# smithzvk/gsl-scattered-interpolation

Hardware: AMD Instinct MI355X
Metric: M interpolated points/sec (whole hot path: fill + solve + eval sweep per step) (higher is better)
Workload: dtype f64; 1 GPU; C3: 3-D N=16384 Gaussian RBF (16k x 16k fp64 Cholesky), M=1M targets per GPU; config=C3, n_centres=16384, dim=3, targets_per_gpu=1000000, targets_total=1000000, parallelism=1 GPU

## Files before the change

gsl-scattered-interpolation_amd/csrc/hip/chol.hip:

```cpp
#include "common.h"
#include <math.h>
#include <stdlib.h>

#ifdef SINTERP_DIAG_PROF
__device__ unsigned long long g_diag_ts[80];
#define TSTAMP(i) do { if (threadIdx.x == 0) g_diag_ts[i] = __builtin_readcyclecounter(); } while (0)
extern "C" int gsl_sinterp_hip_debug_diag_ts(unsigned long long *out) { return (int)hipMemcpyFromSymbol(out, HIP_SYMBOL(g_diag_ts), sizeof(unsigned long long) * 80); }
#endif
#include "chol_potrf.h"
#include "trsm128.h"



__global__ void __launch_bounds__(256)
chol_base_kernel(double *__restrict__ A, size_t lda, size_t n, size_t j0, int nb, int *__restrict__ info,
                 double *__restrict__ diag_store)
{
  __shared__ double sL[CB][CB + 1];
  __shared__ double sInv[CB];
  const int tid = threadIdx.x;

  const size_t row = j0 + nb + (size_t)blockIdx.x * blockDim.x + tid;
  double *p = A + row * lda + j0;
  double x[CB];
// ... 57 lines not shown
    x[j] = v * sInv[j];
  }
  if (vecrow) {
#pragma unroll
    for (int k = 0; k < CB; k += 2) *reinterpret_cast<double2 *>(p + k) = make_double2(x[k], x[k + 1]);
  } else {
#pragma unroll
    for (int k = 0; k < CB; k++) if (k < nb) p[k] = x[k];
  }
}

__global__ void __launch_bounds__(256)
chol_diag_writeback_kernel(double *__restrict__ A, size_t lda, size_t n, const double *__restrict__ diag_store)
{
  const size_t j0 = (size_t)blockIdx.x * CB;
  for (int e = threadIdx.x; e < CB * CB; e += 256) {
    const int r = e / CB, k = e % CB;
    if (k <= r && j0 + r < n) A[(j0 + r) * lda + j0 + k] = diag_store[(size_t)blockIdx.x * (CB * CB) + e];
  }
}


__global__ void __launch_bounds__(256)
chol_diag128_kernel(double *__restrict__ A, size_t lda, size_t j0, int *__restrict__ info, double *__restrict__ diag_store,
                    double *__restrict__ Dinvg, double *__restrict__ fb, size_t ldf, int nrhs)
{
  extern __shared__ __attribute__((aligned(16))) double sm[];
  chol_diag128_block<4>(sm, A + j0 * lda + j0, lda, j0, info, diag_store, Dinvg, fb, ldf, nrhs, threadIdx.x);
}

#define TRX 130
#define TRY 34
template <int RF>
__global__ void __launch_bounds__(256)
chol_trsm16_kernel(double *__restrict__ A, size_t lda, size_t n, size_t j0, const double *__restrict__ Dinvg, size_t row_start,
                   double *__restrict__ fb, size_t ldf, int nrhs)
{
  constexpr bool KSPLIT = RF == 1;
  constexpr int NP = KSPLIT ? 2 : 1;
  constexpr int NRF = KSPLIT ? 1 : RF / 2;
  constexpr int ROWS = 16 * RF;
  constexpr int LCH = KSPLIT ? 4 : 8;
  extern __shared__ __attribute__((aligned(16))) double sm[];
  double *Xp = sm;
  double *Yp = Xp + NP * ROWS * TRX;
  double *ys = Yp + NP * ROWS * TRY;
  const int tid = threadIdx.x, lane = tid & 63, wave = tid >> 6;
  const int f = wave & 1, g = wave >> 1, fr = lane & 15, fq = lane >> 4;
  const int plane = KSPLIT ? g : 0;
  const size_t row0 = row_start + (size_t)blockIdx.x * ROWS;
  const int dch = KSPLIT ? (f ? 4 : 2) : (f ? 8 : 4);
  const int dk0 = KSPLIT ? dch * g : 0, lk0 = KSPLIT ? 4 * g : 0;

  double a0[NRF][8], dv[4][8], lb[6][LCH], yv[3];
  double4_t cinit[NRF][3];
#pragma unroll
  for (int c = 0; c < 4; c++)
#pragma unroll
    for (int i = 0; i < 8; i++) dv[c][i] = i < dch ? Dinvg[c * 1024 + (16 * f + fr) * 32 + 4 * (dk0 + i) + fq] : 0.0;
#pragma unroll
  for (int c = 1; c < 4; c++)
#pragma unroll
    for (int p = 0; p < c; p++)
#pragma unroll
      for (int i = 0; i < LCH; i++)
        lb[c * (c - 1) / 2 + p][i] = A[(j0 + 32 * c + 16 * f + fr) * lda + j0 + 32 * p + 4 * (lk0 + i) + fq];
#pragma unroll
  for (int t = 0; t < NRF; t++) {
    const int rf = KSPLIT ? 0 : g + 2 * t;
    const size_t arow = row0 + 16 * rf + fr < n ? row0 + 16 * rf + fr : n - 1;
    const double *Arow = A + arow * lda + j0;
#pragma unroll
    for (int i = 0; i < 8; i++) a0[t][i] = i < dch ? Arow[4 * (dk0 + i) + fq] : 0.0;
#pragma unroll
    for (int c = 1; c < 4; c++)
#pragma unroll
      for (int rg = 0; rg < 4; rg++) {
        const size_t r = row0 + 16 * rf + fq + 4 * rg < n ? row0 + 16 * rf + fq + 4 * rg : n - 1;
        cinit[t][c - 1][rg] = plane == 0 ? A[r * lda + j0 + 32 * c + 16 * f + fr] : 0.0;
      }
  }
#pragma unroll
  for (int t = 0; t < 3; t++) { const int e = t * 256 + tid; yv[t] = e < nrhs * PB ? fb[(size_t)(e >> 7) * ldf + j0 + (e & 127)] : 0.0; }
#pragma unroll
  for (int t = 0; t < 3; t++) { const int e = t * 256 + tid; if (e < nrhs * PB) ys[e] = yv[t]; }

  double facc[RF][TRSV_MAXR];
#pragma unroll
  for (int t = 0; t < RF; t++)
#pragma unroll
    for (int q = 0; q < TRSV_MAXR; q++) facc[t][q] = 0.0;
  const int sr = tid >> 4, sc = (tid & 15) * 2;

#pragma unroll
  for (int c = 0; c < 4; c++) {
    if (c > 0) {
#pragma unroll
      for (int t = 0; t < NRF; t++) {
        const int rf = KSPLIT ? 0 : g + 2 * t;
        double4_t acc = cinit[t][c - 1];
#pragma unroll
        for (int p = 0; p < c; p++)
#pragma unroll
          for (int i = 0; i < LCH; i++) {
            const int k = 32 * p + 4 * (lk0 + i) + fq;
            double a = Xp[(16 * rf + fr) * TRX + k];
            if constexpr (KSPLIT) a += Xp[ROWS * TRX + (16 * rf + fr) * TRX + k];
            acc = __builtin_amdgcn_mfma_f64_16x16x4f64(-a, lb[c * (c - 1) / 2 + p][i], acc, 0, 0, 0);
          }
#pragma unroll
        for (int rg = 0; rg < 4; rg++) Yp[plane * ROWS * TRY + (16 * rf + fq + 4 * rg) * TRY + 16 * f + fr] = acc[rg];
      }
      __syncthreads();
    }
#pragma unroll
    for (int t = 0; t < NRF; t++) {
      const int rf = KSPLIT ? 0 : g + 2 * t;
      double4_t x = (double4_t){0.0, 0.0, 0.0, 0.0};
#pragma unroll
      for (int i = 0; i < 8; i++) {
        if (i < dch) {
          const int k = 4 * (dk0 + i) + fq;
          double a = a0[t][i];
          if (c > 0) {
            a = Yp[(16 * rf + fr) * TRY + k];
            if constexpr (KSPLIT) a += Yp[ROWS * TRY + (16 * rf + fr) * TRY + k];
          }
          x = __builtin_amdgcn_mfma_f64_16x16x4f64(a, dv[c][i], x, 0, 0, 0);
        }
      }
#pragma unroll
      for (int rg = 0; rg < 4; rg++) Xp[plane * ROWS * TRX + (16 * rf + fq + 4 * rg) * TRX + 32 * c + 16 * f + fr] = x[rg];
    }
    __syncthreads();
#pragma unroll
    for (int t = 0; t < RF; t++) {
      const int r = sr + 16 * t;
      double2 xv = *reinterpret_cast<const double2 *>(&Xp[r * TRX + 32 * c + sc]);
      if constexpr (KSPLIT) {
        const double2 x1 = *reinterpret_cast<const double2 *>(&Xp[ROWS * TRX + r * TRX + 32 * c + sc]);
        xv.x += x1.x; xv.y += x1.y;
      }
      const size_t grow = row0 + r;
      if (grow < n) *reinterpret_cast<double2 *>(A + grow * lda + j0 + 32 * c + sc) = xv;
#pragma unroll
      for (int q = 0; q < TRSV_MAXR; q++)
        if (q < nrhs) facc[t][q] = fma(xv.y, ys[q * PB + 32 * c + sc + 1], fma(xv.x, ys[q * PB + 32 * c + sc], facc[t][q]));
    }
  }
  if (nrhs > 0) {
#pragma unroll
    for (int t = 0; t < RF; t++) {
      const size_t grow = row0 + sr + 16 * t;
#pragma unroll
      for (int q = 0; q < TRSV_MAXR; q++) {
        if (q < nrhs) {
          double v = facc[t][q];
          v += __shfl_xor(v, 1);
          v += __shfl_xor(v, 2);
          v += __shfl_xor(v, 4);
          v += __shfl_xor(v, 8);
          if ((tid & 15) == 0 && grow < n) fb[(size_t)q * ldf + grow] -= v;
        }
      }
    }
  }
}

template <int RF>
static int launch_trsm16(gsl_sinterp_hip_ctx *ctx, double *A, size_t lda, size_t n, size_t j0, const double *d_linv, size_t row_start,
                         double *fb, size_t ldf, int nrhs)
{
  constexpr int NP = RF == 1 ? 2 : 1;
  const size_t lds = (size_t)(NP * 16 * RF * (TRX + TRY) + TRSV_MAXR * PB) * sizeof(double);
  { int ast = sinterp_func_lds(ctx, (const void *)chol_trsm16_kernel<RF>, (int)lds); if (ast) return ast; }
  const size_t below = n - row_start;
  hipLaunchKernelGGL(chol_trsm16_kernel<RF>, dim3((unsigned)((below + 16 * RF - 1) / (16 * RF))), dim3(256), lds, ctx->stream, A, lda, n, j0,
                     d_linv, row_start, fb, ldf, nrhs);
  return ST_SUCCESS;
}

__global__ void __launch_bounds__(256)
chol_trsm128_kernel(double *__restrict__ A, size_t lda, size_t n, size_t j0, const double *__restrict__ Dinvg, size_t row_start,
                    double *__restrict__ fb, size_t ldf, int nrhs)
{
  extern __shared__ __attribute__((aligned(16))) double sm[];
  double *Bt = sm;
  double *ys = sm + TRSM128_LDS;
  const int tid = threadIdx.x, lane = tid & 63, wave = tid >> 6;
  const int fr = lane & 15, fq = lane >> 4;
  const size_t row0 = row_start + (size_t)blockIdx.x * 64;
  double yv[3];
  trsm128_stage(sm, tid,
                [=](int r) { return A + (row0 + r < n ? row0 + r : n - 1) * lda + j0; },
                [=](int bi, int bj, int r, int k) { return A[(j0 + bi * 32 + r) * lda + j0 + bj * 32 + k]; },
                [=](int b, int r, int k) { return Dinvg[b * 1024 + r * 32 + k]; },
                [=, &yv] {
#pragma unroll
                  for (int t = 0; t < 3; t++) { const int e = t * 256 + tid; yv[t] = e < nrhs * PB ? fb[(size_t)(e >> 7) * ldf + j0 + (e & 127)] : 0.0; }
                });
#pragma unroll
  for (int t = 0; t < 3; t++) { const int e = t * 256 + tid; if (e < nrhs * PB) ys[e] = yv[t]; }
  __syncthreads();
  trsm128_solve(sm, tid, [=](int c, int f, int rg, double v) {
    const size_t grow = row0 + wave * 16 + fq + 4 * rg;
    if (grow < n) A[grow * lda + j0 + c * 32 + f * 16 + fr] = v;
  });
  if (nrhs > 0) {
    __syncthreads();
    const int r = tid >> 2, qd = tid & 3;
    const size_t grow = row0 + r;
    for (int q = 0; q < nrhs; q++) {
      double v = 0.0;
#pragma unroll
      for (int k = 0; k < 32; k++) v = fma(Bt[r * TR_LD + qd * 32 + k], ys[q * PB + qd * 32 + k], v);
      v += __shfl_xor(v, 1);
      v += __shfl_xor(v, 2);
      if (qd == 0 && grow < n) fb[(size_t)q * ldf + grow] -= v;
    }
  }
}


__global__ void __launch_bounds__(256)
tricpy_lower_to_upper_kernel(double *__restrict__ A, size_t lda, size_t n)
{
  __shared__ double tile[32][33];
  const size_t bi = blockIdx.y, bj = blockIdx.x;
  if (bj > bi) return;
  const int tx = threadIdx.x & 31, ty = threadIdx.x >> 5;
  for (int r = ty; r < 32; r += 8) {
    const size_t i = bi * 32 + r, j = bj * 32 + tx;
    tile[r][tx] = (i < n && j < n) ? A[i * lda + j] : 0.0;
  }
  __syncthreads();
  for (int r = ty; r < 32; r += 8) {
    const size_t j = bj * 32 + r, i = bi * 32 + tx;
    if (i < n && j < n && j < i) A[j * lda + i] = tile[tx][r];
  }
}

static size_t chol_split(size_t w)
{
  const size_t unit = w > PB ? PB : CB;
  size_t w1 = ((w / 2 + unit - 1) / unit) * unit;
  if (w1 >= w) w1 = w - unit;
  return w1;
}

static int g_chol_riders_last = 0;
extern "C" int gsl_sinterp_hip_debug_chol_riders(void) { return __atomic_load_n(&g_chol_riders_last, __ATOMIC_RELAXED); }

static bool chol_panel128_on(void) { return !SINTERP_ENV_ONCE("GSL_SINTERP_NO_PANEL128"); }

static bool chol_all128(size_t n, const double *d_a, size_t lda)
{
  return chol_panel128_on() && n % PB == 0 && (lda & 1) == 0 && ((((uintptr_t)d_a) & 15) == 0);
}

static bool chol_rider_applicable(bool all128, size_t n)
{
  return all128 && !SINTERP_ENV_ONCE("GSL_SINTERP_NO_DIAG_RIDER") && n >= 2 * PB;
}

static int chol_panel(gsl_sinterp_hip_ctx *ctx, double *A, size_t lda, size_t n, size_t j0, size_t w, int *d_info,
                      double *d_diag, double *fb, size_t ldf, int nrhs, unsigned *d_cnt, bool diag_done)
{
  int st;
  double *d_linv = d_diag + ((n + CB - 1) / CB) * (CB * CB);
  if (w == PB && chol_panel128_on() && (lda & 1) == 0 && ((((uintptr_t)(A + j0 * lda + j0)) & 15) == 0)) {
    const size_t lds_diag = DIAG128_LDS_BYTES;
    { int ast = sinterp_func_lds(ctx, (const void *)chol_diag128_kernel, (int)lds_diag); if (ast) return ast; }
    if (!diag_done)
      hipLaunchKernelGGL(chol_diag128_kernel, dim3(1), dim3(256), lds_diag, ctx->stream, A, lda, j0, d_info,
                         n % PB == 0 ? (double *)NULL : d_diag, d_linv, fb, ldf, nrhs);
    const size_t below = n - j0 - w;
    if (below) {
      static const int force_rf = sinterp_env_int("GSL_SINTERP_TRSM_RF", 0);
      int ast = 0;
      if (force_rf == 1 || (!force_rf && below <= 4096)) ast = launch_trsm16<1>(ctx, A, lda, n, j0, d_linv, j0 + PB, fb, ldf, nrhs);
      else if (force_rf == 2) ast = launch_trsm16<2>(ctx, A, lda, n, j0, d_linv, j0 + PB, fb, ldf, nrhs);
      else if (force_rf == 4) ast = launch_trsm16<4>(ctx, A, lda, n, j0, d_linv, j0 + PB, fb, ldf, nrhs);
      else {
        const size_t lds_trsm = (size_t)(TRSM128_LDS + TRSV_MAXR * PB) * sizeof(double);
        ast = sinterp_func_lds(ctx, (const void *)chol_trsm128_kernel, (int)lds_trsm);
        if (!ast)
          hipLaunchKernelGGL(chol_trsm128_kernel, dim3((unsigned)((below + 63) / 64)), dim3(256), lds_trsm, ctx->stream, A, lda, n, j0,
                             (const double *)d_linv, j0 + PB, fb, ldf, nrhs);
      }
      if (ast) return ast;
    }
    LAUNCH_CHECK(ctx);
    return ST_SUCCESS;
  }
  if (w <= PB) {
    if (diag_done) return sinterp_fail(ctx, ST_EFAILED, "cholesky: rider on a panel that is not 128 wide", hipSuccess, __FILE__, __LINE__);
    if (fb) return sinterp_fail(ctx, ST_EFAILED, "cholesky: folded forward substitution on a panel that is not 128 wide", hipSuccess, __FILE__, __LINE__);
  }
  if (w <= CB) {
    const size_t below = n - j0 - w;
    const unsigned grid = (unsigned)((below + 255) / 256) + (below == 0 ? 1u : 0u);
// ... 317 lines not shown
  __shared__ double sx[TRSV_MAXR][TS];
  __shared__ double sb[TRSV_MAXR][TS];
  __shared__ double sW[TS][TS + 1];
  const int tid = threadIdx.x, lane = tid & 63, wave = tid >> 6;

  double t[16];
  size_t irow = 0;
  bool have = false;
  const int rsub = lane >> 3, c8 = (lane & 7) * 8;
  if (mode == 1) {
    irow = (size_t)blockIdx.x * 64 + lane;
    have = irow < j0;
#pragma unroll
    for (int jj = 0; jj < 16; jj++)
      t[jj] = (have && wave * 16 + jj < nb) ? T[(j0 + wave * 16 + jj) * ldt + irow] : 0.0;
  } else {
    const size_t base = (mode == 0) ? j0 + nb : 0;
    const size_t limit = (mode == 0) ? n : j0;
#pragma unroll
    for (int pass = 0; pass < 2; pass++) {
      const size_t i = base + ((size_t)blockIdx.x * 2 + pass) * 32 + wave * 8 + rsub;
      const double *row = T + i * ldt + j0 + c8;
#pragma unroll
      for (int k = 0; k < 8; k++) t[pass * 8 + k] = (i < limit && c8 + k < nb) ? row[k] : 0.0;
    }
  }
  const double *D = Dinv + (j0 / TS) * (size_t)(TS * TS);
  for (int e = tid; e < TS * TS; e += 256) {
    const int r = e / TS, c = e % TS;
    sW[r][c] = D[e];
  }
  for (int e = tid; e < nrhs * TS; e += 256) {
    const int r = e / TS, c = e % TS;
    sb[r][c] = c < nb ? b[r * ldb + j0 + c] : 0.0;
  }
  __syncthreads();
  for (int r = wave; r < nrhs; r += 4) {
    double acc = 0.0;
    if (mode == 0) { for (int c = 0; c < TS; c++) acc = fma(sW[lane][c], sb[r][c], acc); }
    else { for (int c = 0; c < TS; c++) acc = fma(sW[c][lane], sb[r][c], acc); }
    sx[r][lane] = acc;
    if (blockIdx.x == 0 && lane < nb) xout[r * ldb + j0 + lane] = acc;
  }
  __syncthreads();
  if (mode == 1) {
    __shared__ double s_part[TRSV_MAXR][4][64];
#pragma unroll
    for (int r = 0; r < TRSV_MAXR; r++) {
      if (r < nrhs) {
        double acc = 0.0;
#pragma unroll
        for (int jj = 0; jj < 16; jj++) acc = fma(t[jj], sx[r][wave * 16 + jj], acc);
        s_part[r][wave][lane] = acc;
      }
    }
    __syncthreads();
    if (wave == 0 && have) {
#pragma unroll
      for (int r = 0; r < TRSV_MAXR; r++)
        if (r < nrhs) b[r * ldb + irow] -= (s_part[r][0][lane] + s_part[r][1][lane]) + (s_part[r][2][lane] + s_part[r][3][lane]);
    }
  } else {
    const size_t base = (mode == 0) ? j0 + nb : 0;
    const size_t limit = (mode == 0) ? n : j0;
#pragma unroll
    for (int pass = 0; pass < 2; pass++) {
      const size_t i = base + ((size_t)blockIdx.x * 2 + pass) * 32 + wave * 8 + rsub;
#pragma unroll
      for (int r = 0; r < TRSV_MAXR; r++) {
        if (r < nrhs) {
          double a = 0.0;
#pragma unroll
          for (int k = 0; k < 8; k++) a = fma(t[pass * 8 + k], sx[r][c8 + k], a);
          a += __shfl_xor(a, 1);
          a += __shfl_xor(a, 2);
          a += __shfl_xor(a, 4);
          if (i < limit && (lane & 7) == 0) b[r * ldb + i] -= a;
        }
      }
    }
  }
}

__global__ void __launch_bounds__(256)
trsv_dataflow_kernel(const double *__restrict__ T, size_t ldt, size_t n, const double *__restrict__ b, double *xout, size_t ldb,
                     int nrhs, int mode, const double *__restrict__ Dinv, unsigned *tf, unsigned long long *xq, unsigned nblk)
{
  const unsigned want = __hip_atomic_load(tf, __ATOMIC_RELAXED, __HIP_MEMORY_SCOPE_AGENT) + 1u;
  const size_t npad = (size_t)nblk * TS;
  __shared__ double sx[2][TRSV_MAXR][TS];
  __shared__ double sW[TS][TS + 1];
  __shared__ double srhs[TRSV_MAXR][TS];
  __shared__ double s_part[TRSV_MAXR][4][TS];
  const int tid = threadIdx.x, lane = tid & 63, wave = tid >> 6;
  const int rsub = lane >> 3, c8 = (lane & 7) * 8;
  for (unsigned t = blockIdx.x; t < nblk; t += gridDim.x) {
    const unsigned I = (mode == 0) ? t : nblk - 1 - t;
    const size_t i0 = (size_t)I * TS;
    const int nbI = (int)((n - i0) < TS ? (n - i0) : TS);
    __syncthreads();
    for (int e = tid; e < TS * TS; e += 256) sW[e / TS][e % TS] = Dinv[(size_t)I * (TS * TS) + e];
    double bpre[(TRSV_MAXR * TS + 255) / 256];
#pragma unroll
    for (int q = 0; q < (TRSV_MAXR * TS + 255) / 256; q++) {
      const int e = q * 256 + tid, r = e / TS, c = e % TS;
      bpre[q] = (e < nrhs * TS && c < nbI) ? b[r * ldb + i0 + c] : 0.0;
    }
    double acc[TRSV_MAXR][2];
#pragma unroll
    for (int r = 0; r < TRSV_MAXR; r++) acc[r][0] = acc[r][1] = 0.0;
    for (unsigned sstep = 0; sstep < t; sstep++) {
      const unsigned J = (mode == 0) ? sstep : nblk - 1 - sstep;
      const size_t j0 = (size_t)J * TS;
      double tt[16];
      if (mode == 1) {
#pragma unroll
        for (int jj = 0; jj < 16; jj++) {
          const size_t jr = j0 + wave * 16 + jj;
          tt[jj] = (jr < n && lane < nbI) ? T[jr * ldt + i0 + lane] : 0.0;
        }
      } else {
#pragma unroll
        for (int pass = 0; pass < 2; pass++) {
          const size_t i = i0 + pass * 32 + wave * 8 + rsub;
          const double *row = T + i * ldt + j0 + c8;
          if (i < n && j0 + TS <= n && ((((uintptr_t)row) & 15) == 0)) {
#pragma unroll
            for (int k = 0; k < 8; k += 2) { const double2 v = *reinterpret_cast<const double2 *>(row + k); tt[pass * 8 + k] = v.x; tt[pass * 8 + k + 1] = v.y; }
          } else {
#pragma unroll
            for (int k = 0; k < 8; k++) tt[pass * 8 + k] = (i < n && j0 + c8 + k < n) ? row[k] : 0.0;
          }
        }
      }
      const int buf = sstep & 1;
      for (int e = tid; e < nrhs * TS; e += 256) {
        const int r = e / TS, c = e % TS;
        double v = 0.0;
        if (j0 + c < n) {
          const unsigned long long *q = xq + 2 * ((size_t)r * npad + j0 + c);
          unsigned long long w0, w1;
          for (;;) {
            w0 = __hip_atomic_load(q, __ATOMIC_RELAXED, __HIP_MEMORY_SCOPE_AGENT);
            w1 = __hip_atomic_load(q + 1, __ATOMIC_RELAXED, __HIP_MEMORY_SCOPE_AGENT);
            if ((unsigned)(w0 >> 32) == want && (unsigned)(w1 >> 32) == want) break;
            __builtin_amdgcn_s_sleep(1);
          }
          v = __hiloint2double((int)(unsigned)w1, (int)(unsigned)w0);
        }
        sx[buf][r][c] = v;
      }
      __syncthreads();
      if (mode == 1) {
#pragma unroll
        for (int r = 0; r < TRSV_MAXR; r++)
          if (r < nrhs) {
#pragma unroll
            for (int jj = 0; jj < 16; jj++) acc[r][0] = fma(tt[jj], sx[buf][r][wave * 16 + jj], acc[r][0]);
          }
      } else {
#pragma unroll
        for (int r = 0; r < TRSV_MAXR; r++)
          if (r < nrhs) {
#pragma unroll
            for (int pass = 0; pass < 2; pass++)
#pragma unroll
              for (int k = 0; k < 8; k++) acc[r][pass] = fma(tt[pass * 8 + k], sx[buf][r][c8 + k], acc[r][pass]);
          }
      }
    }
    if (mode == 1) {
#pragma unroll
      for (int r = 0; r < TRSV_MAXR; r++) if (r < nrhs) s_part[r][wave][lane] = acc[r][0];
      __syncthreads();
#pragma unroll
      for (int q = 0; q < (TRSV_MAXR * TS + 255) / 256; q++) {
        const int e = q * 256 + tid, r = e / TS, c = e % TS;
        if (e < nrhs * TS) {
          const double sum = (s_part[r][0][c] + s_part[r][1][c]) + (s_part[r][2][c] + s_part[r][3][c]);
          srhs[r][c] = (c < nbI) ? bpre[q] - sum : 0.0;
        }
      }
    } else {
#pragma unroll
      for (int r = 0; r < TRSV_MAXR; r++)
        if (r < nrhs) {
#pragma unroll
          for (int pass = 0; pass < 2; pass++) {
            double a = acc[r][pass];
            a += __shfl_xor(a, 1);
            a += __shfl_xor(a, 2);
            a += __shfl_xor(a, 4);
            const int row = pass * 32 + wave * 8 + rsub;
            if ((lane & 7) == 0) srhs[r][row] = -a;
          }
        }
      __syncthreads();
#pragma unroll
      for (int q = 0; q < (TRSV_MAXR * TS + 255) / 256; q++) {
        const int e = q * 256 + tid, r = e / TS, c = e % TS;
        if (e < nrhs * TS) srhs[r][c] = (c < nbI) ? bpre[q] + srhs[r][c] : 0.0;
      }
    }
    __syncthreads();
    for (int r = wave; r < nrhs; r += 4) {
      double p0 = 0.0, p1 = 0.0, p2 = 0.0, p3 = 0.0;
      if (mode == 0) {
#pragma unroll
        for (int c = 0; c < TS; c += 4) {
          p0 = fma(sW[lane][c], srhs[r][c], p0); p1 = fma(sW[lane][c + 1], srhs[r][c + 1], p1);
          p2 = fma(sW[lane][c + 2], srhs[r][c + 2], p2); p3 = fma(sW[lane][c + 3], srhs[r][c + 3], p3);
        }
      } else {
#pragma unroll
        for (int c = 0; c < TS; c += 4) {
          p0 = fma(sW[c][lane], srhs[r][c], p0); p1 = fma(sW[c + 1][lane], srhs[r][c + 1], p1);
          p2 = fma(sW[c + 2][lane], srhs[r][c + 2], p2); p3 = fma(sW[c + 3][lane], srhs[r][c + 3], p3);
        }
      }
      if (lane < nbI) {
        const double xv = (p0 + p1) + (p2 + p3);
        unsigned long long *q = xq + 2 * ((size_t)r * npad + i0 + lane);
        const unsigned long long tag = (unsigned long long)want << 32;
        __hip_atomic_store(q, tag | (unsigned)__double2loint(xv), __ATOMIC_RELAXED, __HIP_MEMORY_SCOPE_AGENT);
        __hip_atomic_store(q + 1, tag | (unsigned)__double2hiint(xv), __ATOMIC_RELAXED, __HIP_MEMORY_SCOPE_AGENT);
        xout[r * ldb + i0 + lane] = xv;
      }
    }
    if (t == nblk - 1) {
      __syncthreads();
      if (tid == 0) __hip_atomic_store(tf, want, __ATOMIC_RELAXED, __HIP_MEMORY_SCOPE_AGENT);
    }
  }
}

static int trsv_launches(gsl_sinterp_hip_ctx *ctx, size_t n, const double *T, size_t ldt, double *b, double *xout,
                         size_t ldb, int nrhs, int mode, int unit, double *d_inv, int inv_ready)
{
  const size_t nblk = (n + TS - 1) / TS;
  const bool use_inv = nblk > 1 && d_inv != NULL;
  if (use_inv && !inv_ready) {
    hipLaunchKernelGGL(tri_inv_kernel, dim3((unsigned)nblk), dim3(64), 0, ctx->stream, T, ldt, n, mode == 2 ? 1 : 0, unit, d_inv);
    LAUNCH_CHECK(ctx);
  }
  const bool no_df = SINTERP_ENV_ONCE("GSL_SINTERP_NO_DATAFLOW_TRSV");
  if (use_inv && !no_df && ctx->sk_wgs > 0 && ctx->d_tf && ctx->tf_count >= nblk + 1 && ctx->d_xq) {
    const unsigned G = (unsigned)(nblk < (size_t)ctx->sk_wgs ? nblk : (size_t)ctx->sk_wgs);
    hipLaunchKernelGGL(trsv_dataflow_kernel, dim3(G), dim3(256), 0, ctx->stream, T, ldt, n, (const double *)b, xout, ldb, nrhs, mode,
                       (const double *)d_inv, ctx->d_tf, ctx->d_xq, (unsigned)nblk);
    LAUNCH_CHECK(ctx);
    return ST_SUCCESS;
  }
  for (size_t t = 0; t < nblk; t++) {
    const size_t blk = (mode == 0) ? t : nblk - 1 - t;
    const size_t j0 = blk * TS;
    const int nb = (int)((n - j0) < TS ? (n - j0) : TS);
    const size_t rest = (mode == 0) ? n - j0 - nb : j0;
    const unsigned grid = (unsigned)((rest + 63) / 64);
    if (use_inv)
      hipLaunchKernelGGL(trsv_sweep_inv_kernel, dim3(grid ? grid : 1), dim3(256), 0, ctx->stream, T, ldt, n, b, xout, ldb, nrhs,
                         j0, nb, mode, (const double *)d_inv);
    else
      hipLaunchKernelGGL(trsv_sweep_kernel, dim3(grid ? grid : 1), dim3(256), 0, ctx->stream, T, ldt, n, b, xout, ldb, nrhs, j0,
                         nb, mode, unit);
    LAUNCH_CHECK(ctx);
  }
  return ST_SUCCESS;
}

__global__ void __launch_bounds__(256)
vec_copy_kernel(const double *__restrict__ src, double *__restrict__ dst, size_t count)
{
  const size_t i = (size_t)blockIdx.x * 256 + threadIdx.x;
  if (i < count) dst[i] = src[i];
}

static int trsv_multi_ex(gsl_sinterp_hip_ctx *ctx, size_t n, const double *T, size_t ldt, double *b, double *xout, size_t ldb,
                         int nrhs, int mode, int unit, int inv_ready)
{
  if (n == 0 || nrhs == 0) return ST_SUCCESS;
  if (nrhs > TRSV_MAXR) return sinterp_fail(ctx, ST_EINVAL, "trsv: too many right-hand sides", hipSuccess, __FILE__, __LINE__);
  const int slot = mode == 0 ? 2 : 3;
  const sinterp_graph_key gkey = {{n, ldt, (uintptr_t)T, (uintptr_t)b, (uintptr_t)xout, ldb, (uintptr_t)nrhs, (uintptr_t)mode,
                                    (uintptr_t)unit, (uintptr_t)inv_ready}};
  int replayed = 0;
  int st = sinterp_graph_try_launch(ctx, slot, gkey, &replayed);
  if (st || replayed) return st;
  void *d_inv = NULL;
  const size_t inv_bytes = ((n + TS - 1) / TS) * TS * TS * sizeof(double);
  const bool in_place = b == xout;
  if (in_place && inv_ready) return sinterp_fail(ctx, ST_EINVAL, "trsv: in-place sweep cannot reuse inverted blocks", hipSuccess, __FILE__, __LINE__);
  st = sinterp_invbuf(ctx, inv_bytes + (in_place ? (size_t)nrhs * ldb * sizeof(double) : 0), &d_inv);
  if (st) return st;
  {
    const size_t need = (n + TS - 1) / TS + 1;
    if (need > ctx->tf_count) {
      HIP_OK(ctx, hipStreamSynchronize(ctx->stream));
      if (ctx->d_tf) { HIP_OK(ctx, hipFree(ctx->d_tf)); ctx->d_tf = NULL; ctx->tf_count = 0; }
      const size_t cnt = need < 1024 ? 1024 : need * 2;
      HIP_OK(ctx, hipMalloc((void **)&ctx->d_tf, cnt * sizeof(unsigned)));
      HIP_OK(ctx, hipMemset(ctx->d_tf, 0, cnt * sizeof(unsigned)));
      if (ctx->d_xq) { HIP_OK(ctx, hipFree(ctx->d_xq)); ctx->d_xq = NULL; }
      const size_t xq_bytes = (size_t)TRSV_MAXR * cnt * TS * 2 * sizeof(unsigned long long);
      HIP_OK(ctx, hipMalloc((void **)&ctx->d_xq, xq_bytes));
      HIP_OK(ctx, hipMemset(ctx->d_xq, 0, xq_bytes));
      HIP_OK(ctx, hipDeviceSynchronize());
      ctx->tf_count = cnt;
      for (int i = 2; i < 4; i++)
        if (ctx->graph[i].exec) { (void)hipGraphExecDestroy(ctx->graph[i].exec); ctx->graph[i].exec = NULL; }
    }
  }
  st = sinterp_streamk_prepare(ctx);
  if (st) return st;
  double *b_src = in_place ? (double *)((char *)d_inv + inv_bytes) : b;
  hipStream_t saved;
  st = sinterp_capture_begin(ctx, &saved);
  if (st) return st;
  if (in_place) {
    const size_t cnt = (size_t)(nrhs - 1) * ldb + n;
    hipLaunchKernelGGL(vec_copy_kernel, dim3((unsigned)((cnt + 255) / 256)), dim3(256), 0, ctx->stream, (const double *)b, b_src, cnt);
  }
  st = trsv_launches(ctx, n, T, ldt, b_src, xout, ldb, nrhs, mode, unit, (double *)d_inv, inv_ready);
  int st2 = sinterp_capture_end(ctx, saved, slot, gkey);
  return st ? st : st2;
}

int sinterp_trsv_multi(gsl_sinterp_hip_ctx *ctx, size_t n, const double *T, size_t ldt, double *b, double *xout, size_t ldb,
                       int nrhs, int mode, int unit)
{
  return trsv_multi_ex(ctx, n, T, ldt, b, xout, ldb, nrhs, mode, unit, 0);
}

int sinterp_trsv(gsl_sinterp_hip_ctx *ctx, size_t n, const double *T, size_t ldt, double *b, double *xout, int mode,
                 int unit)
{
  return sinterp_trsv_multi(ctx, n, T, ldt, b, xout, n, 1, mode, unit);
}

int sinterp_cholesky_svx_multi(gsl_sinterp_hip_ctx *ctx, size_t n, const double *d_llt, size_t lda, double *d_x, size_t ldx,
                               int nrhs)
{
  EXCLUSIVE_SECTION(ctx);
  void *d_tmp = NULL;
  int st = sinterp_workspace(ctx, (size_t)nrhs * ldx * sizeof(double), &d_tmp);
  if (st) return st;
  st = sinterp_trsv_multi(ctx, n, d_llt, lda, d_x, (double *)d_tmp, ldx, nrhs, 0, 0);
  if (st) return st;
  return trsv_multi_ex(ctx, n, d_llt, lda, (double *)d_tmp, d_x, ldx, nrhs, 1, 0, 1);
}

extern "C" int gsl_sinterp_hip_cholesky_svx(gsl_sinterp_hip_ctx *ctx, size_t n, const double *d_llt, size_t lda, double *d_x)
{
  REQUIRE(ctx, ctx != NULL, ST_EFAULT);
  HIP_OK(ctx, hipSetDevice(ctx->device));
  EXCLUSIVE_SECTION(ctx);
  REQUIRE(ctx, lda >= n, ST_EINVAL);
  REQUIRE(ctx, n == 0 || (d_llt && d_x), ST_EFAULT);
  return sinterp_cholesky_svx_multi(ctx, n, d_llt, lda, d_x, n, 1);
}
```

gsl-scattered-interpolation_amd/csrc/hip/chol_potrf.h:

```cpp
#ifndef SINTERP_CHOL_POTRF_H
#define SINTERP_CHOL_POTRF_H

#define CB 32
#ifndef TSTAMP
#define TSTAMP(i) do { } while (0)
#endif
#if defined(SINTERP_DIAG_PROF_COLS)
#define TSTAMP_COL(i) TSTAMP(i)
#else
#define TSTAMP_COL(i) do { } while (0)
#endif

__device__ __forceinline__ double lane_bcast(double v, int src)
{
  int lo = __builtin_amdgcn_readlane(__double2loint(v), src);
  int hi = __builtin_amdgcn_readlane(__double2hiint(v), src);
  return __hiloint2double(hi, lo);
}

typedef double double4_t __attribute__((ext_vector_type(4)));
#define PB 128
#define PQ 34
#define PBLK (32 * PQ)
#define TR_LD 130
// ... 27 lines not shown
#define PIN_SSV(x, y, z)   asm volatile("" : "+s"(x), "+s"(y), "+v"(z) : : "memory")
#define PIN_SV(x, y)       asm volatile("" : "+s"(x), "+v"(y) : : "memory")

#define HB 16
template <int K0, int J>
__device__ __forceinline__ void potrf32_step(double (&a)[CB], double vprev, double cur, double inv_prev, double e, double e2, double q,
                                             const double *D, double *colp, const double (&rp)[CB])
{
  constexpr int END = K0 + HB;
  if constexpr (J < END) {
    TSTAMP_COL(32 + J);
    double v, d, uL2 = 0.0, acol = 0.0;
    if constexpr (J == K0) {
      v = cur;
      d = lane_bcast(v, J);
    } else {
      const double uL = e * inv_prev;
      d = fma(-uL, uL, q);
      acol = vprev * inv_prev;
      v = fma(-acol, uL, cur);
      uL2 = e2 * inv_prev;
    }
    double y0 = __builtin_amdgcn_rsq(d);
    PIN_V4(y0, v, uL2, acol);
    if constexpr (J > K0) { a[J - 1] = acol; colp[J - 1] = acol; }
    double rn[CB];
    if constexpr (J + 2 < END) {
#pragma unroll
      for (int k = K0; k < J; k += 2) {
        const double2 t2 = *reinterpret_cast<const double2 *>(D + (J + 2) * PQ + k);
        rn[k] = t2.x;
        if (k + 1 < CB) rn[k + 1] = t2.y;
      }
    }
    double en = 0.0, e2n = 0.0, qn = 0.0, curn = 0.0;
    if constexpr (J + 1 < END) en = lane_bcast(v, J + 1);
    if constexpr (J + 2 < END) e2n = lane_bcast(v, J + 2);
    if constexpr (J + 1 < END) {
      double p0 = a[J + 1], p1 = 0.0;
      if constexpr (J >= K0 + 1) p1 = -acol * uL2;
      PIN_SSV(en, e2n, p0);
#pragma unroll
      for (int k = K0; k + 1 < J; k++) {
        if (k & 1) p1 = fma(-a[k], rp[k], p1);
        else p0 = fma(-a[k], rp[k], p0);
      }
      curn = (J >= K0 + 1) ? p0 + p1 : p0;
      qn = lane_bcast(curn, J + 1);
      PIN_SV(qn, y0);
    }
    const double t = d * y0;
    const double rr = fma(-t, y0, 1.0);
    const double s1 = fma(0.375, rr, 0.5), u = y0 * rr;
    const double inv = fma(u, s1, y0);
    potrf32_step<K0, J + 1>(a, v, curn, inv, en, e2n, qn, D, colp, rn);
  } else {
    a[END - 1] = vprev * inv_prev;
    colp[END - 1] = a[END - 1];
  }
}

__device__ __forceinline__ void potrf32_split(double *D, double *Dt, int lane)
{
  const int fr = lane & 15, fq = lane >> 4;
  const double *ap = D + (HB + fr) * PQ + fq;
  const double *bp = Dt + fr * PQ + fq;
  double4_t cu, cw = (double4_t){0.0, 0.0, 0.0, 0.0};
#pragma unroll
  for (int rg = 0; rg < 4; rg++) cu[rg] = D[(HB + fq + 4 * rg) * PQ + HB + fr];
#pragma unroll
  for (int kk = 0; kk < 4; kk++) {
    const double av = ap[kk * 4], na = -av;
    cu = __builtin_amdgcn_mfma_f64_16x16x4f64(na, av, cu, 0, 0, 0);
    cw = __builtin_amdgcn_mfma_f64_16x16x4f64(na, bp[kk * 4], cw, 0, 0, 0);
  }
#pragma unroll
  for (int rg = 0; rg < 4; rg++) {
    D[(HB + fq + 4 * rg) * PQ + HB + fr] = cu[rg];
    Dt[fr * PQ + HB + fq + 4 * rg] = cw[rg];
  }
}


template <int NW>
__device__ __forceinline__ void potrf128_lds(double *S, double *Dv, int tid, int *__restrict__ info, size_t j0)
{
  const int lane = tid & 63, wave = tid >> 6;
  auto potrf_block = [&](int jb) {
    double *D = S + pblk(jb, jb);
    const bool is_row = lane < CB;
    double *Dt = Dv + jb * PBLK;
    double *colp = is_row ? D + lane * PQ : Dt + (lane - CB) * PQ;
    double a[CB];
#pragma unroll
    for (int k = 0; k < CB; k += 2) { const double2 t = *reinterpret_cast<const double2 *>(colp + k); a[k] = t.x; a[k + 1] = t.y; }
    double r0[CB];
    potrf32_step<0, 0>(a, 0.0, a[0], 0.0, 0.0, 0.0, 0.0, D, colp, r0);
    potrf32_split(D, Dt, lane);
#pragma unroll
    for (int k = HB; k < CB; k += 2) { const double2 t = *reinterpret_cast<const double2 *>(colp + k); a[k] = t.x; a[k + 1] = t.y; }
    potrf32_step<HB, HB>(a, 0.0, a[HB], 0.0, 0.0, 0.0, 0.0, D, colp, r0);
    const double dg = D[(lane & (CB - 1)) * PQ + (lane & (CB - 1))];
    const unsigned long long badm = __ballot(is_row && !(dg > 0.0));
    if (badm && lane == 0) atomicCAS(info, 0, (int)(j0 + jb * 32 + __ffsll((long long)badm)));
  };
  auto update_frag = [&](int jb, int bi, int bj, int f) {
    double *Cb = S + pblk(bi, bj);
    double4_t c = frag_load(Cb, f >> 1, f & 1, lane);
    c = frag_nt(S + pblk(bi, jb), S + pblk(bj, jb), f >> 1, f & 1, lane, c, -1.0);
    frag_store(Cb, f >> 1, f & 1, lane, c);
  };

  for (int jb = -1; jb < 3; jb++) {
    if (jb >= 0) {
    for (int u = wave; u < (3 - jb) * 2; u += NW) {
      double *Bb = S + pblk(jb + 1 + (u >> 1), jb);
      const int fi = u & 1;
      const double *ap = Bb + (fi * 16 + (lane & 15)) * PQ + (lane >> 4);
      const double *bp = Dv + jb * PBLK + (lane >> 4) * PQ + (lane & 15);
      double4_t x0 = (double4_t){0.0, 0.0, 0.0, 0.0}, x1 = x0;
#pragma unroll
      for (int kk = 0; kk < 8; kk++) {
        const double av = ap[kk * 4];
        if (kk < 4) x0 = __builtin_amdgcn_mfma_f64_16x16x4f64(av, bp[kk * 4 * PQ], x0, 0, 0, 0);
        x1 = __builtin_amdgcn_mfma_f64_16x16x4f64(av, bp[kk * 4 * PQ + 16], x1, 0, 0, 0);
      }
      frag_store(Bb, fi, 0, lane, x0);
      frag_store(Bb, fi, 1, lane, x1);
    }
    __syncthreads();
    TSTAMP(4 + jb * 4);
    if (wave < 3) update_frag(jb, jb + 1, jb + 1, wave == 0 ? 0 : wave + 1);
    __syncthreads();
    TSTAMP(5 + jb * 4);
    }
    if (wave == 0) {
      potrf_block(jb + 1);
    } else if (jb >= 0) {
      int unit = 0;
      for (int bi = jb + 2; bi < 4; bi++)
        for (int bj = jb + 1; bj <= bi; bj++)
          for (int f = 0; f < 4; f++) {
            if (bi == bj && f == 1) continue;
            if (unit++ % (NW - 1) == wave - 1) update_frag(jb, bi, bj, f);
          }
    }
    __syncthreads();
    TSTAMP(6 + jb * 4);
  }

}

#ifndef TRSV_MAXR
#define TRSV_MAXR 5
#endif

template <int NW>
__device__ __forceinline__ void diag128_forward(const double *S, const double *Dv, double *fs, double *tt, int tid, int nrhs)
{
  const int lane = tid & 63, wave = tid >> 6, r = lane & 31, half = lane >> 5;
  for (int q = wave; q < nrhs; q += NW) {
    double *y = fs + q * PB, *t = tt + q * CB;
#pragma unroll
    for (int i = 0; i < 4; i++) {
      double sum = 0.0;
#pragma unroll
      for (int kb = 0; kb < i; kb++) {
        const double *Lr = S + pblk(i, kb) + r * PQ + half * 16;
        const double *yk = y + kb * 32 + half * 16;
#pragma unroll
        for (int k = 0; k < 16; k += 2) {
          const double2 l2 = *reinterpret_cast<const double2 *>(Lr + k);
          sum = fma(l2.x, yk[k], sum);
          sum = fma(l2.y, yk[k + 1], sum);
        }
      }
      sum += __shfl_xor(sum, 32);
      if (half == 0) t[r] = y[i * 32 + r] - sum;
      __builtin_amdgcn_wave_barrier();
      const double *Wr = Dv + i * PBLK + (half * 16) * PQ + r;
      double acc = 0.0;
#pragma unroll
      for (int c = 0; c < 16; c++) acc = fma(Wr[c * PQ], t[half * 16 + c], acc);
      acc += __shfl_xor(acc, 32);
      if (half == 0) y[i * 32 + r] = acc;
      __builtin_amdgcn_wave_barrier();
    }
  }
}

#define DIAG128_LDS_BYTES ((size_t)(14 * PBLK + TRSV_MAXR * (PB + CB)) * sizeof(double))

template <int NW>
__device__ __forceinline__ void chol_diag128_block(double *sm, double *Ab, size_t lda, size_t j0, int *info, double *diag_store,
                                                   double *Dinvg, double *fb, size_t ldf, int nrhs, int tid)
{
  constexpr int NT = NW * 64;
  constexpr int RP = NT / 32;
  constexpr int PS = 32 / RP;
  constexpr int FT = (TRSV_MAXR * PB + NT - 1) / NT;
  static_assert(RP * PS == 32, "threads per workgroup");
  double *S = sm;
  double *Dv = S + 10 * PBLK;
  double *fs = Dv + 4 * PBLK;
  double *tt = fs + TRSV_MAXR * PB;
  TSTAMP(0);

  {
    double v[10 * PS], fv[FT];
    const int r8 = tid >> 5, k = tid & 31;
#pragma unroll
    for (int t = 0; t < 10 * PS; t++) {
      constexpr int BI[10] = {0, 1, 1, 2, 2, 2, 3, 3, 3, 3}, BJ[10] = {0, 0, 1, 0, 1, 2, 0, 1, 2, 3};
      const int b = t / PS, r = (t % PS) * RP + r8;
      v[t] = Ab[(size_t)(BI[b] * 32 + r) * lda + BJ[b] * 32 + k];
    }
#pragma unroll
    for (int t = 0; t < FT; t++) { const int e = t * NT + tid; fv[t] = e < nrhs * PB ? fb[(size_t)(e >> 7) * ldf + j0 + (e & 127)] : 0.0; }
#pragma unroll
    for (int t = 0; t < 10 * PS; t++) S[(t / PS) * PBLK + ((t % PS) * RP + r8) * PQ + k] = v[t];
#pragma unroll
    for (int t = 0; t < 4 * PS; t++) { const int r = (t % PS) * RP + r8; Dv[(t / PS) * PBLK + r * PQ + k] = r == k ? 1.0 : 0.0; }
#pragma unroll
    for (int t = 0; t < FT; t++) { const int e = t * NT + tid; if (e < nrhs * PB) fs[e] = fv[t]; }
  }
  __syncthreads();
  TSTAMP(1);

  potrf128_lds<NW>(S, Dv, tid, info, j0);

  TSTAMP(18);
  if (nrhs > 0) {
    diag128_forward<NW>(S, Dv, fs, tt, tid, nrhs);
    __syncthreads();
  }
  {
    const int r8 = tid >> 5, k = tid & 31;
#pragma unroll
    for (int t = 0; t < 10 * PS; t++) {
      constexpr int BI[10] = {0, 1, 1, 2, 2, 2, 3, 3, 3, 3}, BJ[10] = {0, 0, 1, 0, 1, 2, 0, 1, 2, 3};
      const int b = t / PS, r = (t % PS) * RP + r8, bi = BI[b], bj = BJ[b];
      const double v = S[b * PBLK + r * PQ + k];
      if (bi != bj || k <= r) Ab[(size_t)(bi * 32 + r) * lda + bj * 32 + k] = v;
      if (bi == bj && diag_store) diag_store[(j0 / CB + bi) * (CB * CB) + r * CB + k] = (k <= r) ? v : 0.0;
    }
#pragma unroll
    for (int t = 0; t < 4 * PS; t++) {
      const int b = t / PS, r = (t % PS) * RP + r8;
      Dinvg[b * 1024 + r * 32 + k] = Dv[b * PBLK + k * PQ + r];
    }
#pragma unroll
    for (int t = 0; t < FT; t++) { const int e = t * NT + tid; if (e < nrhs * PB) fb[(size_t)(e >> 7) * ldf + j0 + (e & 127)] = fs[e]; }
  }
  TSTAMP(19);
}

#endif
```

Measured before the change: 33.21 M points/s.

## Overlap diagonal forward solve with potrf and prefetch RHS in trsm kernels

Interleaves the per-block forward substitution for the right-hand sides into the potrf128 pipeline, so idle waves run it while wave 0 factors the next diagonal block. The trsm16 and trsm128 kernels now prefetch the RHS values early and write them back directly instead of doing a read-modify-write at the end. The in-place vector copy is skipped when the dataflow TRSV path applies. The dataflow kernel also gains a bounded spin with an abort flag that writes NaN if polling times out. This adds complexity and ties correctness to the abort_word scratch slot and the removed __restrict__ on b.

```diff
diff --git a/gsl-scattered-interpolation_amd/csrc/hip/chol.hip b/gsl-scattered-interpolation_amd/csrc/hip/chol.hip
--- a/gsl-scattered-interpolation_amd/csrc/hip/chol.hip
+++ b/gsl-scattered-interpolation_amd/csrc/hip/chol.hip
@@ -163,6 +163,12 @@
   }
 #pragma unroll
   for (int t = 0; t < 3; t++) { const int e = t * 256 + tid; yv[t] = e < nrhs * PB ? fb[(size_t)(e >> 7) * ldf + j0 + (e & 127)] : 0.0; }
+  double fv[RF][TRSV_MAXR];
+#pragma unroll
+  for (int t = 0; t < RF; t++)
+#pragma unroll
+    for (int q = 0; q < TRSV_MAXR; q++)
+      fv[t][q] = ((tid & 15) == 0 && q < nrhs && row0 + (tid >> 4) + 16 * t < n) ? fb[(size_t)q * ldf + row0 + (tid >> 4) + 16 * t] : 0.0;
 #pragma unroll
   for (int t = 0; t < 3; t++) { const int e = t * 256 + tid; if (e < nrhs * PB) ys[e] = yv[t]; }
 
@@ -241,7 +247,7 @@
           v += __shfl_xor(v, 2);
           v += __shfl_xor(v, 4);
           v += __shfl_xor(v, 8);
-          if ((tid & 15) == 0 && grow < n) fb[(size_t)q * ldf + grow] -= v;
+          if ((tid & 15) == 0 && grow < n) fb[(size_t)q * ldf + grow] = fv[t][q] - v;
         }
       }
     }
@@ -272,13 +278,17 @@
   const int fr = lane & 15, fq = lane >> 4;
   const size_t row0 = row_start + (size_t)blockIdx.x * 64;
   double yv[3];
+  double fv[TRSV_MAXR];
+  const bool fown = (tid & 3) == 0 && row0 + (tid >> 2) < n;
   trsm128_stage(sm, tid,
                 [=](int r) { return A + (row0 + r < n ? row0 + r : n - 1) * lda + j0; },
                 [=](int bi, int bj, int r, int k) { return A[(j0 + bi * 32 + r) * lda + j0 + bj * 32 + k]; },
                 [=](int b, int r, int k) { return Dinvg[b * 1024 + r * 32 + k]; },
-                [=, &yv] {
+                [=, &yv, &fv] {
 #pragma unroll
                   for (int t = 0; t < 3; t++) { const int e = t * 256 + tid; yv[t] = e < nrhs * PB ? fb[(size_t)(e >> 7) * ldf + j0 + (e & 127)] : 0.0; }
+#pragma unroll
+                  for (int q = 0; q < TRSV_MAXR; q++) fv[q] = (fown && q < nrhs) ? fb[(size_t)q * ldf + row0 + (tid >> 2)] : 0.0;
                 });
 #pragma unroll
   for (int t = 0; t < 3; t++) { const int e = t * 256 + tid; if (e < nrhs * PB) ys[e] = yv[t]; }
@@ -291,13 +301,16 @@
     __syncthreads();
     const int r = tid >> 2, qd = tid & 3;
     const size_t grow = row0 + r;
-    for (int q = 0; q < nrhs; q++) {
-      double v = 0.0;
-#pragma unroll
-      for (int k = 0; k < 32; k++) v = fma(Bt[r * TR_LD + qd * 32 + k], ys[q * PB + qd * 32 + k], v);
-      v += __shfl_xor(v, 1);
-      v += __shfl_xor(v, 2);
-      if (qd == 0 && grow < n) fb[(size_t)q * ldf + grow] -= v;
+#pragma unroll
+    for (int q = 0; q < TRSV_MAXR; q++) {
+      if (q < nrhs) {
+        double v = 0.0;
+#pragma unroll
+        for (int k = 0; k < 32; k++) v = fma(Bt[r * TR_LD + qd * 32 + k], ys[q * PB + qd * 32 + k], v);
+        v += __shfl_xor(v, 1);
+        v += __shfl_xor(v, 2);
+        if (fown) fb[(size_t)q * ldf + grow] = fv[q] - v;
+      }
     }
   }
 }
@@ -781,9 +794,11 @@
   }
 }
 
+#define TRSV_MAX_POLLS (1u << 22)
 __global__ void __launch_bounds__(256)
-trsv_dataflow_kernel(const double *__restrict__ T, size_t ldt, size_t n, const double *__restrict__ b, double *xout, size_t ldb,
-                     int nrhs, int mode, const double *__restrict__ Dinv, unsigned *tf, unsigned long long *xq, unsigned nblk)
+trsv_dataflow_kernel(const double *__restrict__ T, size_t ldt, size_t n, const double *b, double *xout, size_t ldb,
+                     int nrhs, int mode, const double *__restrict__ Dinv, unsigned *tf, unsigned long long *xq, unsigned nblk,
+                     unsigned *abort_word)
 {
   const unsigned want = __hip_atomic_load(tf, __ATOMIC_RELAXED, __HIP_MEMORY_SCOPE_AGENT) + 1u;
   const size_t npad = (size_t)nblk * TS;
@@ -791,8 +806,10 @@
   __shared__ double sW[TS][TS + 1];
   __shared__ double srhs[TRSV_MAXR][TS];
   __shared__ double s_part[TRSV_MAXR][4][TS];
+  __shared__ unsigned s_dead;
   const int tid = threadIdx.x, lane = tid & 63, wave = tid >> 6;
   const int rsub = lane >> 3, c8 = (lane & 7) * 8;
+  if (tid == 0) s_dead = 0u;
   for (unsigned t = blockIdx.x; t < nblk; t += gridDim.x) {
     const unsigned I = (mode == 0) ? t : nblk - 1 - t;
     const size_t i0 = (size_t)I * TS;
@@ -838,14 +855,20 @@
         double v = 0.0;
         if (j0 + c < n) {
           const unsigned long long *q = xq + 2 * ((size_t)r * npad + j0 + c);
-          unsigned long long w0, w1;
-          for (;;) {
+          unsigned long long w0 = 0ull, w1 = 0ull;
+          bool lost = *(volatile unsigned *)&s_dead != 0u;
+          for (unsigned spins = 0; !lost; spins++) {
             w0 = __hip_atomic_load(q, __ATOMIC_RELAXED, __HIP_MEMORY_SCOPE_AGENT);
             w1 = __hip_atomic_load(q + 1, __ATOMIC_RELAXED, __HIP_MEMORY_SCOPE_AGENT);
             if ((unsigned)(w0 >> 32) == want && (unsigned)(w1 >> 32) == want) break;
+            if (spins >= TRSV_MAX_POLLS) {
+              lost = true;
+              *(volatile unsigned *)&s_dead = 1u;
+              __hip_atomic_store(abort_word, 1u, __ATOMIC_RELAXED, __HIP_MEMORY_SCOPE_AGENT);
+            }
             __builtin_amdgcn_s_sleep(1);
           }
-          v = __hiloint2double((int)(unsigned)w1, (int)(unsigned)w0);
+          v = lost ? __longlong_as_double(0x7ff8000000000000ll) : __hiloint2double((int)(unsigned)w1, (int)(unsigned)w0);
         }
         sx[buf][r][c] = v;
       }
@@ -933,6 +956,13 @@
   }
 }
 
+static bool trsv_dataflow_applicable(gsl_sinterp_hip_ctx *ctx, size_t n, const double *d_inv)
+{
+  const size_t nblk = (n + TS - 1) / TS;
+  return nblk > 1 && d_inv != NULL && !SINTERP_ENV_ONCE("GSL_SINTERP_NO_DATAFLOW_TRSV") && ctx->sk_wgs > 0 && ctx->d_tf &&
+         ctx->tf_count >= nblk + 1 && ctx->d_xq;
+}
+
 static int trsv_launches(gsl_sinterp_hip_ctx *ctx, size_t n, const double *T, size_t ldt, double *b, double *xout,
                          size_t ldb, int nrhs, int mode, int unit, double *d_inv, int inv_ready)
 {
@@ -942,11 +972,11 @@
     hipLaunchKernelGGL(tri_inv_kernel, dim3((unsigned)nblk), dim3(64), 0, ctx->stream, T, ldt, n, mode == 2 ? 1 : 0, unit, d_inv);
     LAUNCH_CHECK(ctx);
   }
-  const bool no_df = SINTERP_ENV_ONCE("GSL_SINTERP_NO_DATAFLOW_TRSV");
-  if (use_inv && !no_df && ctx->sk_wgs > 0 && ctx->d_tf && ctx->tf_count >= nblk + 1 && ctx->d_xq) {
+  if (trsv_dataflow_applicable(ctx, n, d_inv)) {
     const unsigned G = (unsigned)(nblk < (size_t)ctx->sk_wgs ? nblk : (size_t)ctx->sk_wgs);
+    unsigned *abort_word = (unsigned *)((int *)ctx->d_scratch + 8 + 1);
     hipLaunchKernelGGL(trsv_dataflow_kernel, dim3(G), dim3(256), 0, ctx->stream, T, ldt, n, (const double *)b, xout, ldb, nrhs, mode,
-                       (const double *)d_inv, ctx->d_tf, ctx->d_xq, (unsigned)nblk);
+                       (const double *)d_inv, ctx->d_tf, ctx->d_xq, (unsigned)nblk, abort_word);
     LAUNCH_CHECK(ctx);
     return ST_SUCCESS;
   }
@@ -1011,11 +1041,12 @@
   }
   st = sinterp_streamk_prepare(ctx);
   if (st) return st;
-  double *b_src = in_place ? (double *)((char *)d_inv + inv_bytes) : b;
+  const bool copy = in_place && !trsv_dataflow_applicable(ctx, n, (const double *)d_inv);
+  double *b_src = copy ? (double *)((char *)d_inv + inv_bytes) : b;
   hipStream_t saved;
   st = sinterp_capture_begin(ctx, &saved);
   if (st) return st;
-  if (in_place) {
+  if (copy) {
     const size_t cnt = (size_t)(nrhs - 1) * ldb + n;
     hipLaunchKernelGGL(vec_copy_kernel, dim3((unsigned)((cnt + 255) / 256)), dim3(256), 0, ctx->stream, (const double *)b, b_src, cnt);
   }
diff --git a/gsl-scattered-interpolation_amd/csrc/hip/chol_potrf.h b/gsl-scattered-interpolation_amd/csrc/hip/chol_potrf.h
--- a/gsl-scattered-interpolation_amd/csrc/hip/chol_potrf.h
+++ b/gsl-scattered-interpolation_amd/csrc/hip/chol_potrf.h
@@ -133,8 +133,49 @@
 }
 
 
+#ifndef TRSV_MAXR
+#define TRSV_MAXR 5
+#endif
+
+__device__ __forceinline__ void diag128_forward_sum(const double *S, double *fs, double *tt, int lane, int q, int i)
+{
+  const int r = lane & 31, half = lane >> 5;
+  double *y = fs + q * PB, *t = tt + q * CB;
+  double sum = 0.0;
+#pragma unroll
+  for (int kb = 0; kb < 3; kb++) {
+    if (kb < i) {
+      const double *Lr = S + pblk(i, kb) + r * PQ + half * 16;
+      const double *yk = y + kb * 32 + half * 16;
+#pragma unroll
+      for (int k = 0; k < 16; k += 2) {
+        const double2 l2 = *reinterpret_cast<const double2 *>(Lr + k);
+        sum = fma(l2.x, yk[k], sum);
+        sum = fma(l2.y, yk[k + 1], sum);
+      }
+    }
+  }
+  sum += __shfl_xor(sum, 32);
+  if (half == 0) t[r] = y[i * 32 + r] - sum;
+  __builtin_amdgcn_wave_barrier();
+}
+
+__device__ __forceinline__ void diag128_forward_inv(const double *Dv, double *fs, double *tt, int lane, int q, int i)
+{
+  const int r = lane & 31, half = lane >> 5;
+  double *y = fs + q * PB, *t = tt + q * CB;
+  const double *Wr = Dv + i * PBLK + (half * 16) * PQ + r;
+  double acc = 0.0;
+#pragma unroll
+  for (int c = 0; c < 16; c++) acc = fma(Wr[c * PQ], t[half * 16 + c], acc);
+  acc += __shfl_xor(acc, 32);
+  if (half == 0) y[i * 32 + r] = acc;
+  __builtin_amdgcn_wave_barrier();
+}
+
 template <int NW>
-__device__ __forceinline__ void potrf128_lds(double *S, double *Dv, int tid, int *__restrict__ info, size_t j0)
+__device__ __forceinline__ void potrf128_lds(double *S, double *Dv, int tid, int *__restrict__ info, size_t j0,
+                                             double *fs, double *tt, int nrhs)
 {
   const int lane = tid & 63, wave = tid >> 6;
   auto potrf_block = [&](int jb) {
@@ -187,57 +228,25 @@
     }
     if (wave == 0) {
       potrf_block(jb + 1);
-    } else if (jb >= 0) {
-      int unit = 0;
-      for (int bi = jb + 2; bi < 4; bi++)
-        for (int bj = jb + 1; bj <= bi; bj++)
-          for (int f = 0; f < 4; f++) {
-            if (bi == bj && f == 1) continue;
-            if (unit++ % (NW - 1) == wave - 1) update_frag(jb, bi, bj, f);
-          }
+    } else {
+      if (jb >= 0) {
+        int unit = 0;
+        for (int bi = jb + 2; bi < 4; bi++)
+          for (int bj = jb + 1; bj <= bi; bj++)
+            for (int f = 0; f < 4; f++) {
+              if (bi == bj && f == 1) continue;
+              if (unit++ % (NW - 1) == wave - 1) update_frag(jb, bi, bj, f);
+            }
+      }
+      for (int q = wave - 1; q < nrhs; q += NW - 1) {
+        if (jb >= 0) diag128_forward_inv(Dv, fs, tt, lane, q, jb);
+        diag128_forward_sum(S, fs, tt, lane, q, jb + 1);
+      }
     }
     __syncthreads();
     TSTAMP(6 + jb * 4);
   }
 
-}
-
-#ifndef TRSV_MAXR
-#define TRSV_MAXR 5
-#endif
-
-template <int NW>
-__device__ __forceinline__ void diag128_forward(const double *S, const double *Dv, double *fs, double *tt, int tid, int nrhs)
-{
-  const int lane = tid & 63, wave = tid >> 6, r = lane & 31, half = lane >> 5;
-  for (int q = wave; q < nrhs; q += NW) {
-    double *y = fs + q * PB, *t = tt + q * CB;
-#pragma unroll
-    for (int i = 0; i < 4; i++) {
-      double sum = 0.0;
-#pragma unroll
-      for (int kb = 0; kb < i; kb++) {
-        const double *Lr = S + pblk(i, kb) + r * PQ + half * 16;
-        const double *yk = y + kb * 32 + half * 16;
-#pragma unroll
-        for (int k = 0; k < 16; k += 2) {
-          const double2 l2 = *reinterpret_cast<const double2 *>(Lr + k);
-          sum = fma(l2.x, yk[k], sum);
-          sum = fma(l2.y, yk[k + 1], sum);
-        }
-      }
-      sum += __shfl_xor(sum, 32);
-      if (half == 0) t[r] = y[i * 32 + r] - sum;
-      __builtin_amdgcn_wave_barrier();
-      const double *Wr = Dv + i * PBLK + (half * 16) * PQ + r;
-      double acc = 0.0;
-#pragma unroll
-      for (int c = 0; c < 16; c++) acc = fma(Wr[c * PQ], t[half * 16 + c], acc);
-      acc += __shfl_xor(acc, 32);
-      if (half == 0) y[i * 32 + r] = acc;
-      __builtin_amdgcn_wave_barrier();
-    }
-  }
 }
 
 #define DIAG128_LDS_BYTES ((size_t)(14 * PBLK + TRSV_MAXR * (PB + CB)) * sizeof(double))
@@ -278,11 +287,11 @@
   __syncthreads();
   TSTAMP(1);
 
-  potrf128_lds<NW>(S, Dv, tid, info, j0);
+  potrf128_lds<NW>(S, Dv, tid, info, j0, fs, tt, nrhs);
 
   TSTAMP(18);
   if (nrhs > 0) {
-    diag128_forward<NW>(S, Dv, fs, tt, tid, nrhs);
+    for (int q = tid >> 6; q < nrhs; q += NW) diag128_forward_inv(Dv, fs, tt, tid & 63, q, 3);
     __syncthreads();
   }
   {
```

New measurement: 33.46 M points/s (median of 6 runs). No clear change (+0.8%).
